# xiaohong-huang/RTK-Visual-Inertial-Navigation

Measured on AMD Instinct MI355X. Metric: gauss_newton_iterations_per_sec, higher is better.
Workload: dtype f64; 1 GPU; BASELINE cfg4: batch of 512 independent cfg3 windows (20 keyframes, 300 features, 3000 observations, 19 IMU factors, 10 satellites x 20 epochs carrier-phase+pseudorange, gauge prior) over the job, 8 dogleg iterations per solve; windows=512, windows_rank0=512

## Files before the change

### rtk_visual_inertial_navigation_amd/build.py

```python
import os
import subprocess

HERE = os.path.dirname(os.path.abspath(__file__))
CSRC = os.path.join(HERE, "csrc")
LIB = os.path.join(HERE, "libswf_hip.so")
SOURCES = ["swf_engine.hip", "swf_plan.cpp", "swf_problem.cpp", "swf_producers.hip", "swf_gnss_epochs.cpp", "swf_lambda.hip", "swf_features.hip", "swf_fixprior.hip", "swf_phasescreen.hip", "swf_gnssepoch.hip", "swf_ddselect.hip", "swf_pnp.hip", "swf_trackreject.hip"]
HEADERS = ["swf_dev.h", "swf_records.h", "swf_plan.h", "swf_kernels.h", "swf_clique_mm.h", "swf_lmschur.h", "swf_chol_rr4.h", "swf_kernels2.h", "swf_kernels3.h", "swf_rootdev.h", "swf_kernels4.h", "swf_lambda.h", "swf_features.h", "swf_fixprior.h", "swf_gnss_range.h", "swf_phasescreen.h", "swf_gnssepoch.h", "swf_ddselect.h", "swf_pnp.h", "swf_trackreject.h",
           os.path.join("..", "..", "include", "swf_types.h"),
           os.path.join("..", "..", "include", "swf_solver.h")]


def hipcc():
    for p in (os.environ.get("HIPCC"), "/opt/rocm/bin/hipcc", "hipcc"):
        if p and (os.path.isabs(p) and os.path.exists(p) or not os.path.isabs(p)):
            return p
    return "hipcc"


def needs_build():
    if not os.path.exists(LIB):
        return True
    t = os.path.getmtime(LIB)
    for f in SOURCES + HEADERS:
        p = os.path.join(CSRC, f)
        if os.path.exists(p) and os.path.getmtime(p) > t:
            return True
    return False


def build(force=False, verbose=False):
# ... 14 lines not shown
```

### rtk_visual_inertial_navigation_amd/csrc/swf_engine.hip

```cpp
#include <hip/hip_runtime.h>
#include <algorithm>
#include <chrono>
#include <cmath>
#include <cstdio>
#include <cstdlib>
#include <cstring>
#include <string>
#include <memory>
#include <thread>
#include <vector>
#include "../../include/swf_solver.h"
#include "swf_kernels2.h"
#include "swf_kernels3.h"
#include "swf_kernels4.h"
#include "swf_lambda.h"
#include "swf_ddselect.h"
#include "swf_features.h"
#include "swf_fixprior.h"
#include "swf_plan.h"

static thread_local std::string g_err;
static int fail(int code, const std::string& msg) { g_err = msg; return code; }
#define HIPCHK(x) do { hipError_t e_ = (x); if (e_ != hipSuccess) return fail(SWF_E_NODEVICE, std::string(#x) + ": " + hipGetErrorString(e_)); } while (0)

// ... 186 lines not shown
    std::vector<double> h_fxA, h_fxb, h_fxJ, h_fxr0, h_fxeig, h_fxx0; std::vector<int> h_fxrank, h_fxapplied;
    bool fc_built = false, fc_valid = false, fc_host = false; FeatArgs fc{}; char* fc_out = nullptr; size_t fc_bytes = 0; int fc_nfeat = 0;
    std::vector<int> fc_feat0; std::vector<char> h_fc;
    hipStream_t aux = nullptr; hipEvent_t ev_fork[3] = { nullptr, nullptr, nullptr };
    ~swf_batch() {
        if (aux) { (void)hipStreamSynchronize(aux); handle_cache().give(aux); }
        for (auto& e : ev_fork) handle_cache().give(e, false);
    }
    WinState* ws_primary = nullptr; WinState* ws_alt = nullptr; WinState* ws_alt2 = nullptr;
    bool no_decide_fuse = false;
    bool no_step_fuse = false;
    int n_pch_split = 0;
    bool no_spec = false;
    bool no_comp_fuse = false;
    bool lat_fuse = false;
    bool rr4_has15 = false, rr4_has16 = false;
    int rr_nmax = 256;
    bool L_full = false;
    int asm_programs = 0;
    int ls_qpb = 1, ls_var = 0, ls_kms = 8; bool ls_folded = false, s_direct = false;
    bool full_final = false;
    bool no_clq_pack = false;
    bool no_clq_mfma = false;
    int clp_rows = 1, clp_ld = 3;
    int ls_gqpb = 4;
    int timing = 0;
    swf_timing last{};
    std::vector<hipEvent_t> ev;
    std::vector<int> ev_kind;
    int ev_used = 0;
    int64_t jac_bytes = 0, proj_bytes = 0, chol_flops = 0, lm_schur_flops = 0, lm_schur_flops_sym = 0, lm_schur_mfma = 0;
    int last_mode = -1;
};

extern "C" int swf_batch_create(const swf_flat_window* const* windows, int32_t n, void* stream, swf_batch** out) {
    if (!windows || n <= 0 || !out) return fail(SWF_E_INVALID, "swf_batch_create: bad arguments");
    int ndev = 0;
    if (hipGetDeviceCount(&ndev) != hipSuccess || ndev <= 0)
        return fail(SWF_E_NODEVICE, "no HIP device: this library has no CPU fallback");
    int n_cu = 256;
    { int dev = 0; hipDeviceProp_t pr; if (hipGetDevice(&dev) == hipSuccess && hipGetDeviceProperties(&pr, dev) == hipSuccess && pr.multiProcessorCount > 0) n_cu = pr.multiProcessorCount; }
    Plan B;
    {
        std::string err;
        int prc = plan_build(windows, n, plan_shape_from_env(n_cu), B, err);
        if (prc != SWF_OK) return fail(prc, err);
    }
    std::unique_ptr<swf_batch> owner(new swf_batch());
    swf_batch* b = owner.get();
    b->device = current_device();
    b->stream = (hipStream_t)stream;
    b->n_cu = n_cu;
    b->no_comp_fuse = getenv("SWF_NO_COMP_FUSE") != nullptr;
    b->no_spec = getenv("SWF_NO_SPEC_EVAL") != nullptr;
    b->no_step_fuse = getenv("SWF_NO_STEP_FUSE") != nullptr;
    b->no_decide_fuse = getenv("SWF_NO_DECIDE_FUSE") != nullptr;
    b->full_final = getenv("SWF_FULL_FINAL_ELIM") != nullptr;
    b->no_clq_pack = getenv("SWF_NO_CLIQUE_PACK") != nullptr;
    b->no_clq_mfma = getenv("SWF_NO_CLIQUE_MFMA") != nullptr;
    b->max_tiles = B.max_tiles; b->max_prior_dim = B.max_prior_dim; b->max_red = B.max_red; b->min_red = B.min_red;
    b->rr_nmax = B.rr_nmax; b->rr4_has15 = B.rr4_has15; b->rr4_has16 = B.rr4_has16; b->n_pch_split = B.n_pch_split;
    b->lat_fuse = B.lat_fuse; b->asm_programs = B.asm_programs;
    b->ls_qpb = B.ls_qpb; b->ls_var = B.ls_var; b->ls_kms = B.ls_kms; b->ls_gqpb = B.ls_gqpb; b->ls_folded = B.ls_folded; b->s_direct = B.s_direct;
    for (int k = 0; k < 5; k++) b->clc_imu[k] = B.clc_imu[k];
    b->clp_rows = B.clp_rows; b->clp_ld = B.clp_ld;
    b->n_comp = B.n_comp; b->comp_nmax = B.comp_nmax; b->comp_nmin = B.comp_nmin; b->comp_ne = B.comp_ne;
    b->jac_bytes = B.jac_bytes; b->proj_bytes = B.proj_bytes; b->chol_flops = B.chol_flops;
    b->lm_schur_flops = B.lm_schur_flops; b->lm_schur_flops_sym = B.lm_schur_flops_sym; b->lm_schur_mfma = B.lm_schur_mfma;
    if (B.want_aux) {
        bool ok = (b->aux = handle_cache().stream()) != nullptr;
        for (int i = 0; i < 3 && ok; i++) ok = (b->ev_fork[i] = handle_cache().event(false)) != nullptr;
        if (!ok) { handle_cache().give(b->aux); b->aux = nullptr; }
    }
    DevBatch& D = b->D;
    DevPool& P = b->pool;
    int rc = 0;
    D.n_win = n; D.n_x = (int)B.n_x; D.n_loc_total = (int)B.n_loc; D.max_iter_trace = SWF_MAX_TRACE; D.rr_nmax = B.rr_nmax;
    D.n_lmb = B.n_lmb; D.n_pch = B.n_pch; D.n_proj = B.n_proj; D.n_lm = B.n_lm; D.n_fr = B.n_fr; D.n_fsb = B.n_fsb;
    D.n_gf = (int)B.gf.size(); D.n_imu = (int)B.imu_gf.size(); D.n_sc = (int)B.sc_gf.size(); D.n_prior = (int)B.prior_gf.size(); D.n_idp = (int)B.idp_gf.size();
    D.n_cl = (int)B.cl.size(); D.n_pair = (int)B.pair.size(); D.n_pd = B.n_pd; D.n_po = B.n_po; D.n_cle = B.n_cle;
    for (int k = 0; k < 5; k++) D.n_clc[k] = B.n_clc[k];
    D.as_max_ne = B.as_max_ne; D.as_max_nv = B.as_max_nv;
#define PUT(field) rc |= P.put(B.field, &D.field)
    PUT(win);
    PUT(lmb_rec); PUT(pch_q); PUT(pch_r0); PUT(prior_nch);
    PUT(blk_xoff); PUT(blk_loc); PUT(blk_gs);
    PUT(loc2x); PUT(x_var);
    PUT(p_win); PUT(p_xpose); PUT(p_xex); PUT(p_xlm);
// ... 184 lines not shown
    if (!b) return fail(SWF_E_INVALID, "null batch");
    b->fc_valid = false; b->dd_valid = false;
    int n = b->D.n_x;
    hipLaunchKernelGGL(k_copy, dim3((n + 255) / 256), dim3(256), 0, b->stream, b->D.x, (const double*)b->D.x0, n);
    HIPCHK(hipGetLastError());
    if (b->n_comp) {
        HIPCHK(hipMemcpyAsync(b->CA.pose, b->co_pose0, (size_t)b->comp_ne * 7 * sizeof(double), hipMemcpyDeviceToDevice, b->stream));
        HIPCHK(hipMemcpyAsync(b->CA.sb, b->co_sb0, (size_t)b->comp_ne * 9 * sizeof(double), hipMemcpyDeviceToDevice, b->stream));
        HIPCHK(hipMemsetAsync(b->CA.history, 0, (size_t)b->n_comp * sizeof(int), b->stream));
    }
    return SWF_OK;
}

static DevOpt to_devopt(const swf_options* o) {
    DevOpt d{};
    d.max_iter = o->max_num_iterations; d.step_mode = o->step_mode; d.strategy = o->trust_region_strategy; d.jacobi = o->jacobi_scaling ? 1 : 0;
    d.r0 = o->initial_trust_region_radius; d.max_r = o->max_trust_region_radius; d.min_r = o->min_trust_region_radius;
    d.min_rel_dec = o->min_relative_decrease; d.ftol = o->function_tolerance; d.gtol = o->gradient_tolerance;
    d.ptol = o->parameter_tolerance; d.min_mu = o->min_mu; d.max_mu = o->max_mu; d.mu_inc = o->mu_increase_factor;
    d.min_diag = o->min_diagonal; d.max_diag = o->max_diagonal;
    return d;
}

#define GRID(n, per) dim3((unsigned)(((n) + (per) - 1) / (per)))
namespace {
struct Launcher {
    swf_batch* b; DevOpt O; hipStream_t st;
    bool lm_folded = false;
    bool export_full = false;
    int lm_next = 0, lm_qpb = 1;
    int ls_tiles_per_launch() const { return b->ls_var == 0 ? 16 : b->ls_var == 1 ? 40 : 72; }
    WinState* ws_next(WinState* p) const { return p == b->ws_primary ? b->ws_alt : p == b->ws_alt ? b->ws_alt2 : b->ws_primary; }
    bool decide_fused = false;
    void lm_launch(int tile_base, hipStream_t on, int clique_rows = 0) {
        DevBatch& D = b->D;
        dim3 grid(D.n_win, GEMM_SPLIT / b->ls_qpb);
        const int qpb = b->ls_qpb, sd = b->s_direct ? 1 : 0, lp = tile_base / ls_tiles_per_launch(), kms = b->ls_kms;
        if (clique_rows > 0) {
            const int np = (int)grid.y;
            grid.y += clique_rows;
            if (decide_fused) {
                WinState* out = ws_next(D.ws);
                if (b->ls_var == 0) hipLaunchKernelGGL((k_decide_lm_clique<8, 2, 2, 80>), grid, dim3(LS_NT(8, 2)), 0, on, D, O, qpb, lp, kms, sd, np, out);
                else hipLaunchKernelGGL((k_decide_lm_clique<8, 5, 2, 144>), grid, dim3(LS_NT(8, 2)), 0, on, D, O, qpb, lp, kms, sd, np, out);
                D.ws = out;
                return;
// ... 128 lines not shown
                hipLaunchKernelGGL((k_lm_schur<8, 2, 2, 80, false, true>), grid, dim3(256), 0, st, D, O, b->ls_gqpb, 0, 0, 0);
            } else if (!write_S) {
                dim3 grid(D.n_win, GEMM_SPLIT / lm_qpb);
                hipLaunchKernelGGL((k_lm_schur<8, 2, 2, 80, false>), grid, dim3(256), 0, st, D, O, lm_qpb, 0, 0, 0);
            } else {
                const int crow = D.n_win > 0 ? (D.n_clc[2] + D.n_win - 1) / D.n_win : 0;
                clq_fused = clq_fuse_ok();
                lm_launch(0, st, clq_fused ? crow : 0);
                lm_next = ls_tiles_per_launch();
            }
        }
        {
            hipStream_t sa = b->aux ? b->aux : st;
            if (b->aux) (void)hipStreamWaitEvent(b->aux, b->ev_fork[1], 0);
            auto cstream = [&](int cls) { return (b->aux && !b->clc_imu[cls]) ? st : sa; };
            if (comp_fused) {
                for (; lm_next < b->max_tiles; lm_next += ls_tiles_per_launch()) { Bracket t(*this, SWF_K_LM_SCHUR, sa); lm_launch(lm_next, sa); }
            } else {
            const bool grad = !write_S && !b->full_final;
            if (D.n_clc[1]) {
                Bracket t(*this, SWF_K_CLIQUE_ELIM, cstream(1));
                if (grad) hipLaunchKernelGGL((k_clique_elim<32, 48, 9, 1, true>), dim3(D.n_clc[1]), dim3(64), 0, cstream(1), D, O);
                else if (b->no_clq_mfma) hipLaunchKernelGGL((k_clique_elim<32, 48, 9, 1>), dim3(D.n_clc[1]), dim3(64), 0, cstream(1), D, O);
                else hipLaunchKernelGGL((k_clique_mm<32, 48, 9>), dim3(D.n_clc[1]), dim3(64), 0, cstream(1), D, O);
            }
            if (D.n_clc[0]) {
                Bracket t(*this, SWF_K_CLIQUE_ELIM, cstream(0));
                constexpr int CLP_NW = 1;
                const size_t lds = CLP_NW * 2 * ((size_t)(b->clp_rows + 2) * b->clp_ld + b->clp_rows + 2) * sizeof(double);
                const dim3 cgrid(((D.n_clc[0] + 1) / 2 + CLP_NW - 1) / CLP_NW);
                if (b->no_clq_pack) {
                    if (grad) hipLaunchKernelGGL((k_clique_elim<48, 32, 1, 0, true>), dim3(D.n_clc[0]), dim3(64), 0, cstream(0), D, O);
                    else hipLaunchKernelGGL((k_clique_elim<48, 32, 1, 0>), dim3(D.n_clc[0]), dim3(64), 0, cstream(0), D, O);
                }
                else if (grad) hipLaunchKernelGGL((k_clique_pack<true, CLP_NW>), cgrid, dim3(64 * CLP_NW), lds, cstream(0), D, O, b->clp_rows, b->clp_ld);
                else hipLaunchKernelGGL((k_clique_pack<false, CLP_NW>), cgrid, dim3(64 * CLP_NW), lds, cstream(0), D, O, b->clp_rows, b->clp_ld);
            }
            if (D.n_clc[2] && !clq_fused) {
                Bracket t(*this, SWF_K_CLIQUE_ELIM, cstream(2));
                if (b->lat_fuse) {
                    if (grad) hipLaunchKernelGGL(k_clique_elim4<true>, dim3(D.n_clc[2]), dim3(256), 0, cstream(2), D, O);
                    else hipLaunchKernelGGL(k_clique_elim4<false>, dim3(D.n_clc[2]), dim3(256), 0, cstream(2), D, O);
                }
                else if (grad) hipLaunchKernelGGL((k_clique_elim<64, 64, 9, 2, true>), dim3(D.n_clc[2]), dim3(64), 0, cstream(2), D, O);
                else hipLaunchKernelGGL((k_clique_elim<64, 64, 9, 2>), dim3(D.n_clc[2]), dim3(64), 0, cstream(2), D, O);
            }
// ... 963 lines not shown
    }
    if (!ok) return fail(SWF_E_NODEVICE, "download failed");
    return SWF_OK;
}

extern "C" int swf_debug_plan_check(const swf_flat_window* const* windows, int32_t n, int32_t n_cu, int32_t ls_variant, int32_t ls_qpb, int32_t ls_grad_qpb,
                                    int32_t flags, int32_t corrupt_table, int32_t corrupt_index, int32_t* info) {
    if (!windows || n <= 0 || n_cu <= 0) return fail(SWF_E_INVALID, "swf_debug_plan_check: bad arguments");
    PlanShape sh;
    sh.n_cu = n_cu; sh.ls_variant = ls_variant; sh.ls_qpb = ls_qpb; sh.ls_grad_qpb = ls_grad_qpb; sh.no_lat_fuse = flags & 1; sh.no_chol_col = flags & 2;
    Plan B; std::string err;
    int rc = plan_build(windows, n, sh, B, err);
    if (rc != SWF_OK) return fail(rc, err);
    if (corrupt_table) {
        const size_t i = (size_t)corrupt_index;
        if (corrupt_table == 1 && i < B.as_src.size()) B.as_src[i] += 1 << 28;
        else if (corrupt_table == 2 && i < B.sch_rec.size()) B.sch_rec[i] ^= 1;
        else if (corrupt_table == 3 && i < B.s_tnz.size() && B.s_tnz[i]) B.s_tnz[i] &= B.s_tnz[i] - 1;
        else if (corrupt_table == 4 && i < B.prior_colloc.size()) B.prior_colloc[i] ^= 1;
        else if (corrupt_table == 5 && i < B.loc2x.size()) B.loc2x[i] ^= 1;
        else if (corrupt_table == 6 && i < B.co_voff.size()) B.co_voff[i] += 1 << 28;
        else if (corrupt_table == 7 && i < B.pair_o.size()) B.pair_o[i].q_base += 8;
        else if (corrupt_table == 8 && i < B.imu_rec.size()) B.imu_rec[i].xo[3] ^= 1;
        else return fail(SWF_E_INVALID, "swf_debug_plan_check: nothing to corrupt there");
    }
    if (info) {
        const int v[12] = { B.ls_var, B.ls_qpb, B.ls_gqpb, B.ls_folded, B.lat_fuse, B.want_aux, B.want_Linv, B.want_Wk, B.asm_programs, B.n_pch_split, B.max_red, B.n_pch };
        for (int k = 0; k < 12; k++) info[k] = v[k];
    }
    rc = plan_validate(B, err);
    return rc == SWF_OK ? SWF_OK : fail(rc, err);
}

extern "C" int swf_debug_mfma_f64(const double* A, const double* Bm, const double* C, double* D) {
    if (!A || !Bm || !C || !D) return fail(SWF_E_INVALID, "swf_debug_mfma_f64: bad arguments");
    double* dv = nullptr;
    if (hipMalloc(&dv, (64 + 64 + 256 + 256) * sizeof(double)) != hipSuccess) return fail(SWF_E_NODEVICE, "swf_debug_mfma_f64: allocation failed");
    bool ok = hipMemcpy(dv, A, 64 * sizeof(double), hipMemcpyHostToDevice) == hipSuccess
        && hipMemcpy(dv + 64, Bm, 64 * sizeof(double), hipMemcpyHostToDevice) == hipSuccess
        && hipMemcpy(dv + 128, C, 256 * sizeof(double), hipMemcpyHostToDevice) == hipSuccess;
    if (ok) {
        hipLaunchKernelGGL(k_debug_mfma_f64, dim3(1), dim3(64), 0, 0, dv, dv + 64, dv + 128, dv + 384);
        ok = hipGetLastError() == hipSuccess && hipMemcpy(D, dv + 384, 256 * sizeof(double), hipMemcpyDeviceToHost) == hipSuccess;
    }
    (void)hipFree(dv);
    return ok ? SWF_OK : fail(SWF_E_NODEVICE, "swf_debug_mfma_f64: the device run failed");
}

#ifdef SWF_PROFILE_CHOL
extern "C" int swf_debug_chol_stamps(unsigned long long* out) {
    if (hipDeviceSynchronize() != hipSuccess) return SWF_E_NODEVICE;
    if (hipMemcpyFromSymbol(out, HIP_SYMBOL(g_chol_stamps), 64 * sizeof(unsigned long long)) != hipSuccess) return SWF_E_NODEVICE;
    return SWF_OK;
}
#endif

#ifdef SWF_PROFILE_CHOLW
extern "C" int swf_debug_chol_wstep(int step) {
    if (hipDeviceSynchronize() != hipSuccess) return SWF_E_NODEVICE;
    unsigned long long z[16 * 8] = { 0 };
    if (hipMemcpyToSymbol(HIP_SYMBOL(g_chol_wst), z, sizeof(z)) != hipSuccess) return SWF_E_NODEVICE;
    if (hipMemcpyToSymbol(HIP_SYMBOL(g_chol_wstep), &step, sizeof(int)) != hipSuccess) return SWF_E_NODEVICE;
    return SWF_OK;
}
extern "C" int swf_debug_chol_wstamps(unsigned long long* out) {
    if (hipDeviceSynchronize() != hipSuccess) return SWF_E_NODEVICE;
    if (hipMemcpyFromSymbol(out, HIP_SYMBOL(g_chol_wst), 16 * 8 * sizeof(unsigned long long)) != hipSuccess) return SWF_E_NODEVICE;
    return SWF_OK;
}
// ... 175 lines not shown
```

### rtk_visual_inertial_navigation_amd/csrc/swf_kernels.h

```cpp
#pragma once
#include "swf_dev.h"

struct DevOpt {
    int max_iter, step_mode, strategy, jacobi;
    double r0, max_r, min_r, min_rel_dec, ftol, gtol, ptol, min_mu, max_mu, mu_inc, min_diag, max_diag;
};



__device__ __forceinline__ double damp_diag(const DevOpt& O, double d, double* jsc_slot, bool first) {
    if (!O.jacobi) return clampd(d, O.min_diag, O.max_diag);
    double q;
    if (first) { double r = 1.0 + sqrt(d > 0.0 ? d : 0.0); q = r * r; *jsc_slot = q; }
    else q = *jsc_slot;
    return clampd(d / q, O.min_diag, O.max_diag) * q;
}

__device__ __forceinline__ double pinned_d(double v) { asm volatile("" : "+v"(v)); return v; }
template <bool JAC> __device__ __forceinline__ bool eval_gate(const DevBatch& B, const WinState& s) { return B.spec == 2 ? true : (JAC && !B.spec) ? s.need_lin != 0 : s.eval_cand != 0; }
template <bool JAC> __device__ __forceinline__ const double* eval_src(const DevBatch& B) { return (JAC && !B.spec) ? B.x : B.xc; }

#include "swf_gnss_range.h"

template <bool JAC, bool STORE>
// ... 1056 lines not shown
            }
#pragma unroll
            for (int u = 0; u < 2; u++) {
                if (!on[u]) continue;
                int i = i0[u], j = j0[u];
                bool i1ok = i + 1 < df, j1ok = j + 1 < df;
                Cm[i * df + j] = m[u][0]; Cm[j * df + i] = m[u][0];
                if (i1ok) { Cm[(i + 1) * df + j] = m[u][2]; Cm[j * df + i + 1] = m[u][2]; }
                if (!diag[u] && j1ok) { Cm[i * df + j + 1] = m[u][1]; Cm[(j + 1) * df + i] = m[u][1]; }
                if (i1ok && j1ok) { Cm[(i + 1) * df + j + 1] = m[u][3]; Cm[(j + 1) * df + i + 1] = m[u][3]; }
            }
        }
    }
    QST(5);
}
template <int MAXR, int MAXD, int MAXE, int CLS, bool GRAD = false>
__global__ void __launch_bounds__(64) k_clique_elim(DevBatch B, DevOpt O) { d_clique_elim<MAXR, MAXD, MAXE, CLS, 24, 1, 4, GRAD>(B, O, (int)blockIdx.x); }
template <bool GRAD = false>
__global__ void __launch_bounds__(256) k_clique_elim4(DevBatch B, DevOpt O) { d_clique_elim<64, 64, 9, 2, 8, 4, 4, GRAD>(B, O, (int)blockIdx.x); }
template <bool GRAD = false>
__global__ void __launch_bounds__(256) k_clique_tall(DevBatch B, DevOpt O) { d_clique_elim<CLQ_TALLR, 64, 9, 4, 8, 4, 4, GRAD>(B, O, (int)blockIdx.x); }

#include "swf_clique_mm.h"

__device__ __forceinline__ double readhalf_d(double v, bool upper) { double a = readlane_d(v, 0), b = readlane_d(v, 32); return upper ? b : a; }
template <bool GRAD, int NW>
__global__ void __launch_bounds__(64 * NW) k_clique_pack(DevBatch B, DevOpt O, const int R, const int LD) {
    constexpr int PF = 12;
    extern __shared__ double clp_lds[];
    const int lane = threadIdx.x & 63, hl = lane & 31, pair = (int)blockIdx.x * NW + (NW > 1 ? __builtin_amdgcn_readfirstlane((int)threadIdx.x >> 6) : 0);
    const bool up = lane >= 32;
    double* Jc = clp_lds + (2 * (pair - (int)blockIdx.x * NW) + (up ? 1 : 0)) * ((R + 2) * LD + R + 2);
    double* rv = Jc + R * LD; double* Me = rv + R; double* T = Me + LD; double* Ei = T + LD; double* Eg = Ei + 1;
    const int n = B.n_clc[0];
    int cidx = 2 * pair + (up ? 1 : 0);
    bool act = cidx < n;
    const Clique& C = B.clc_rec[0][act ? cidx : 0];
    WinState& s = B.ws[C.win];
    act = act && s.need_lin;
    if (__builtin_amdgcn_ballot_w64(act) == 0) return;
    const int de = act ? C.d_e : 0, df = act ? C.d_f : 0, d = de + df, nrow = act ? C.n_rows : 0, tot = nrow * d;
    const int nrow_m = max(__builtin_amdgcn_readlane(nrow, 0), __builtin_amdgcn_readlane(nrow, 32));
    const int tot_m = max(__builtin_amdgcn_readlane(tot, 0), __builtin_amdgcn_readlane(tot, 32));
    {
        const double* gJ = B.g_J + C.j_off;
        float rd = 1.0f / (float)(nrow > 0 ? nrow : 1);
// ... 412 lines not shown
```

### rtk_visual_inertial_navigation_amd/csrc/swf_plan.cpp

```cpp
#include <algorithm>
#include <array>
#include <cstdlib>
#include <cstring>
#include <map>
#include <string>
#include <vector>
#include "swf_plan.h"

namespace {
int refuse(std::string& err, int code, const std::string& msg) { err = msg; return code; }
int ls_ncw(int var) { return var <= 1 ? 8 : 12; }
int ls_tpw(int var) { return var == 0 ? 2 : var == 1 ? 5 : 6; }

int plan_window(Plan& B, const swf_flat_window* w, int wi, HostWin& hw, std::string& err) {
    WinRec R{};
    const int nP = w->n_pose, nS = w->n_sb, nL = w->n_lm, nC = w->n_sc;
    const int nb = nP + nS + nL + nC;
    if (nb <= 0) return refuse(err, SWF_E_INVALID, "empty window");
    hw = HostWin{ w->pose, w->sb, w->lm, w->sc, nP, nS, nL, nC, 0 };
    R.x_base = (int)B.n_x; R.blk_base = (int)B.blk_xoff.size(); R.n_blk = nb;
    R.loc_base = (int)B.n_loc;
    std::vector<int> gs(nb), ls(nb), xo(nb), loc(nb, -1), grp(nb, -1);
    int xoff = 0;
    for (int b = 0; b < nb; b++) {
// ... 717 lines not shown
    std::stable_sort(po.begin(), po.end(), [&](int a, int c) {
        return (B.pair[a].la * B.pair[a].lb + 15) / 16 > (B.pair[c].la * B.pair[c].lb + 15) / 16; });
    for (size_t i = 0; i < B.cl.size(); i++) {
        const Clique& c = B.cl[i];
        if (c.d_e > 0) cle.push_back((int)i);
        if (c.is_static) continue;
        int d = c.d_e + c.d_f;
        int cls = (c.d_e <= 1 && d <= 32 && c.n_rows <= 48) ? 0 : (c.n_rows <= 32 && d <= 48) ? 1 : (c.n_rows <= CLQ_MAXR && d <= CLQ_MAXD) ? 2 : (c.n_rows <= CLQ_TALLR && d <= 64) ? 4 : 3;
        if (B.lat_fuse && cls < 2) cls = 2;
        clc[cls].push_back((int)i);
        for (int q = c.fac0; q < c.fac1; q++) if (B.gf[B.cl_fac[q]].type == GF_IMU) B.clc_imu[cls] = true;
    }
    B.n_pd = (int)pd.size(); B.n_po = (int)po.size(); B.n_cle = (int)cle.size();
    std::vector<Pair>&vd = B.pair_d, &vo = B.pair_o;
    for (int i : pd) vd.push_back(B.pair[i]);
    for (int i : po) vo.push_back(B.pair[i]);
    for (int i : cle) B.cle_rec.push_back(B.cl[i]);
    for (int k = 0; k < 5; k++) {
        for (int i : clc[k]) B.clc_rec[k].push_back(B.cl[i]);
        B.n_clc[k] = (int)clc[k].size();
    }
    B.clp_rows = 1; B.clp_ld = 3;
    for (const Clique& c : B.clc_rec[0]) { B.clp_rows = std::max(B.clp_rows, c.n_rows); B.clp_ld = std::max(B.clp_ld, (c.d_e + c.d_f + 2) | 1); }
}

int plan_asm_programs(Plan& B, const std::vector<int>& pd, const std::vector<int>& po, std::string& err) {
    const int n_part = B.s_direct ? 0 : B.ls_folded ? 1 : GEMM_SPLIT, n_qpart = B.ls_folded ? 1 : GEMM_SPLIT;
    const int n = B.n_win;
    struct Prog { std::vector<int> dst, src0, aux, src, vloc, vred, vsrc0, vi, vsrc; std::vector<unsigned> cnt, vcnt; };
    std::vector<AsmWin>& asw = B.asw;
    asw.assign((size_t)n, AsmWin{});
    std::vector<int>&t_dst = B.as_dst, &t_src0 = B.as_src0, &t_aux = B.as_aux, &t_src = B.as_src, &tv_loc = B.av_loc, &tv_red = B.av_red, &tv_src0 = B.av_src0, &tv_i = B.av_i, &tv_src = B.av_src;
    std::vector<unsigned>&t_cnt = B.as_cnt, &tv_cnt = B.av_cnt;
    std::map<std::vector<int>, std::array<int, 4>> seen;
    std::vector<std::vector<int>> wpairs((size_t)n);
    for (int i : pd) wpairs[(size_t)B.pair[i].win].push_back(i);
    for (int i : po) wpairs[(size_t)B.pair[i].win].push_back(i);
    bool overflow = false;
    std::vector<unsigned>& tnz = B.s_tnz;
    tnz.assign((size_t)n * 4, 0u);
    for (const Pair& Pq : B.pair) {
        if (B.win[(size_t)Pq.win].n_red > 256) continue;
        for (int I = Pq.ra / 16; I <= (Pq.ra + Pq.la - 1) / 16; I++)
            for (int J = Pq.rb / 16; J <= (Pq.rb + Pq.lb - 1) / 16 && J < I; J++) { const int t = I * (I - 1) / 2 + J; tnz[(size_t)Pq.win * 4 + (t >> 5)] |= 1u << (t & 31); }
    }
    for (int w = 0; w < n; w++) {
// ... 293 lines not shown
        }
        if (!C.is_static) cl_seen[{ C.fac0, C.mem0, C.e_off }] = 0;
    }
    for (int k = 0; k < 5; k++) {
        NEED((int)B.clc_rec[k].size() == B.n_clc[k], "clc_rec", k);
        for (const Clique& C : B.clc_rec[k]) {
            const long long d = C.d_e + C.d_f; const int R = C.n_rows;
            auto it = cl_seen.find({ C.fac0, C.mem0, C.e_off });
            NEED(it != cl_seen.end() && it->second++ == 0, "clc_rec", k);
            NEED(k == 0 ? (C.d_e <= 1 && d <= 32 && R <= 48) : k == 1 ? (R <= 32 && d <= 48) : k == 2 ? (R <= CLQ_MAXR && d <= CLQ_MAXD) : k == 4 ? (R <= CLQ_TALLR && d <= 64)
                        : (d <= CB_MAXD && C.d_e <= 9 && (long long)C.d_e * d <= CB_MAXED), "clc_rec", k);
        }
    }
    for (auto& kv : cl_seen) NEED(kv.second == 1, "clc_rec: a clique in no class, fac0", kv.first[0]);
    NEED(B.clp_rows >= 1 && B.clp_rows <= 48 && B.clp_ld >= 3 && B.clp_ld <= 35 && (B.clp_ld & 1) == 1, "clp_rows", B.clp_rows);
    {
        int mr = 1, ml = 3;
        for (const Clique& C : B.clc_rec[0]) {
            NEED(C.n_rows <= B.clp_rows && C.d_e + C.d_f + 2 <= B.clp_ld, "clp_ld", &C - B.clc_rec[0].data());
            mr = std::max(mr, C.n_rows); ml = std::max(ml, (C.d_e + C.d_f + 2) | 1);
        }
        NEED(mr == B.clp_rows && ml == B.clp_ld, "clp_rows: not the largest class-0 clique", mr);
    }
    const int TW = B.ls_var <= 1 ? 2 : 1, NCW = ls_ncw(B.ls_var), TPW = ls_tpw(B.ls_var);
    NEED((long long)B.sch_rec.size() >= ((long long)B.sch_c0.back() + 4 * LS_NB) * 32 && (long long)B.sch_km.size() >= ((long long)B.sch_c0.back() / TW + 2) * B.ls_kms, "sch_rec", B.sch_rec.size());
    std::vector<std::vector<const Pair*>> wpair((size_t)n);
    auto pair_ok = [&](const Pair& P) {
        if (!in(P.win, 0, n)) return false;
        const WinRec& W = B.win[P.win];
        return P.ra >= 0 && P.la >= 1 && P.ra + P.la <= W.n_red && P.rb >= 0 && P.lb >= 1 && P.rb + P.lb <= W.n_red && P.rb <= P.ra && in(P.fa, -1, W.nF) && in(P.fb, -1, W.nF)
            && P.c0 >= 0 && P.c0 <= P.c1 && P.c1 <= (long long)B.pc_coff.size() && (P.is_diag ? (P.ra == P.rb && P.la == P.lb) : P.ra != P.rb) && P.loc_a == W.loc_base + W.n_e + P.ra
            && P.fsb0 == W.fsb0 && P.fsb1 == W.fsb1 && P.n == W.n_red && P.m == 6 * W.nF && P.S_base == W.S_base && P.P_base == W.P_base && P.q_base == 6LL * W.fr_base * GEMM_SPLIT;
    };
    NEED((int)B.pair_d.size() == B.n_pd && (int)B.pair_o.size() == B.n_po, "pair_d", B.pair_d.size());
    for (const Pair& P : B.pair) NEED(pair_ok(P), "pair", &P - B.pair.data());
    for (const Pair& P : B.pair_d) { NEED(pair_ok(P) && P.is_diag, "pair_d", &P - B.pair_d.data()); wpair[P.win].push_back(&P); }
    for (const Pair& P : B.pair_o) { NEED(pair_ok(P) && !P.is_diag, "pair_o", &P - B.pair_o.data()); wpair[P.win].push_back(&P); }
    std::map<std::array<int, 4>, std::vector<int>> programs;
    for (int w = 0; w < n; w++) {
        const WinRec& W = B.win[w];
        NEED(W.n_e + W.n_red == W.n_loc && W.loc_base >= 0 && W.loc_base + W.n_loc <= B.n_loc && W.x_base >= 0 && W.x_base + W.x_n <= B.n_x, "win", w);
        NEED(W.S_base >= 0 && W.S_base + (long long)(W.n_red + 1) * W.n_red <= B.S_tot && W.Lt_base + (long long)(W.n_red + 1) * (W.n_red + 1) <= B.Lt_tot && W.P_base + 36LL * W.nF * W.nF <= B.P_tot, "win", w);
        NEED(W.fr_base >= 0 && W.fr_base + W.nF <= B.n_fr && W.nF <= LS_MAXF && W.lm0 <= W.lm1 && W.lm1 <= B.n_lm, "win", w);
        for (int f = 0; f < W.nF; f++) NEED(B.fr_red[W.fr_base + f] >= 0 && B.fr_red[W.fr_base + f] + 6 <= W.n_red, "fr_red", W.fr_base + f);
        {
            int l = W.lm0;
// ... 89 lines not shown
```

### rtk_visual_inertial_navigation_amd/csrc/swf_plan.h

```cpp
#pragma once
#include <string>
#include <vector>
#include "../../include/swf_solver.h"
#include "swf_records.h"

struct FeatWinSrc {
    int x_base = 0, n_pose = 0, n_sb = 0, n_lm = 0, n_sc = 0;
    std::vector<int> proj_idx; std::vector<double> proj_uv;
    std::vector<int> idp_kind, idp_idx; std::vector<double> idp_pts;
    double pbg[3] = { 0, 0, 0 }; double sqrt_info = 0;
};

struct HostWin {
    double *pose, *sb, *lm, *sc;
    int n_pose, n_sb, n_lm, n_sc;
    int tail_dim;
    double *comp_pose = nullptr, *comp_sb = nullptr;
    int comp_e0 = 0, comp_ne = 0;
    std::vector<int> p_orig;
    int n_proj_all = 0;
    std::vector<int> tail_x;
    FeatWinSrc feat;
    struct LinPrior { int gf, dim, gsum; std::vector<int> col_x; };
    std::vector<LinPrior> lin_prior;
// ... 42 lines not shown
    int max_tiles = 0, max_prior_dim = 0;
    std::vector<int> lmb_rec, pch_q, pch_r0, prior_nch;
    std::vector<int> sch_c0, sch_rec, sch_km;
    std::vector<int> fsb_rec;
    std::vector<JtRec> sc_jt, imu_jt;
    std::vector<ImuRec> imu_rec;
    std::vector<double> prior_Jt;
    std::vector<int> prior_colloc, prior_colcc, s_pcol, s_pxo, cv_loc;
    std::vector<Pair> pair_d, pair_o;
    std::vector<Clique> clc_rec[5], cle_rec;
    std::vector<AsmWin> asw;
    std::vector<unsigned> s_tnz;
    std::vector<int> as_dst, as_src0, as_aux, as_src, av_loc, av_red, av_src0, av_i, av_src;
    std::vector<unsigned> as_cnt, av_cnt;
    std::vector<int> co_eo, co_no, co_roff, co_x0off, co_voff, co_iq_f, co_iq_k;
    std::vector<long long> co_pno, co_nno, co_go, co_g2o, co_Joff, co_Coff;
    int n_win = 0, n_proj = 0, n_lm = 0, n_lmb = 0, n_pch = 0, n_fsb = 0, n_pd = 0, n_po = 0, n_cle = 0, n_clc[5] = { 0, 0, 0, 0, 0 };
    int as_max_ne = 0, as_max_nv = 0;
    int n_cu = 256, rr_nmax = 256, max_red = 0, min_red = 1 << 30;
    int ls_qpb = 1, ls_var = 0, ls_kms = 8, ls_gqpb = 4; bool ls_folded = false, s_direct = false;
    bool lat_fuse = false, want_aux = false, want_Linv = false, want_Wk = false;
    bool clc_imu[5] = { false, false, false, false, false };
    int clp_rows = 1, clp_ld = 3;
    int n_pch_split = 0; bool rr4_has15 = false, rr4_has16 = false;
    int n_comp = 0, comp_nmax = 0, comp_nmin = 1 << 30; long long comp_ne = 0;
    int asm_programs = 0;
    int64_t jac_bytes = 0, proj_bytes = 0, chol_flops = 0, lm_schur_flops = 0, lm_schur_flops_sym = 0, lm_schur_mfma = 0;
};

int plan_build(const swf_flat_window* const* windows, int n, const PlanShape& shape, Plan& plan, std::string& err);

int plan_validate(const Plan& plan, std::string& err);
```

Before: 733,300 iterations/s.

## Add direct class-1 clique elimination kernel using augmented-column MFMA Gram

Adds k_clique_md, a class-1 clique elimination kernel that appends the residual as an extra column. One set of f64 MFMA passes then yields both the Gram matrix and the gradient. It inverts the eliminated block in registers with a lane-broadcast Gauss-Jordan and applies the Schur update with MFMA into the same accumulators. The plan picks it when every class-1 clique has at most 47 columns, and an env var turns it off. The aim is fewer passes and less shared-memory traffic per clique, at the cost of extra register pressure and a second code path to keep correct.

```diff
diff --git a/rtk_visual_inertial_navigation_amd/build.py b/rtk_visual_inertial_navigation_amd/build.py
--- a/rtk_visual_inertial_navigation_amd/build.py
+++ b/rtk_visual_inertial_navigation_amd/build.py
@@ -5,7 +5,7 @@
 CSRC = os.path.join(HERE, "csrc")
 LIB = os.path.join(HERE, "libswf_hip.so")
 SOURCES = ["swf_engine.hip", "swf_plan.cpp", "swf_problem.cpp", "swf_producers.hip", "swf_gnss_epochs.cpp", "swf_lambda.hip", "swf_features.hip", "swf_fixprior.hip", "swf_phasescreen.hip", "swf_gnssepoch.hip", "swf_ddselect.hip", "swf_pnp.hip", "swf_trackreject.hip"]
-HEADERS = ["swf_dev.h", "swf_records.h", "swf_plan.h", "swf_kernels.h", "swf_clique_mm.h", "swf_lmschur.h", "swf_chol_rr4.h", "swf_kernels2.h", "swf_kernels3.h", "swf_rootdev.h", "swf_kernels4.h", "swf_lambda.h", "swf_features.h", "swf_fixprior.h", "swf_gnss_range.h", "swf_phasescreen.h", "swf_gnssepoch.h", "swf_ddselect.h", "swf_pnp.h", "swf_trackreject.h",
+HEADERS = ["swf_dev.h", "swf_records.h", "swf_plan.h", "swf_kernels.h", "swf_clique_mm.h", "swf_clique_md.h", "swf_lmschur.h", "swf_chol_rr4.h", "swf_kernels2.h", "swf_kernels3.h", "swf_rootdev.h", "swf_kernels4.h", "swf_lambda.h", "swf_features.h", "swf_fixprior.h", "swf_gnss_range.h", "swf_phasescreen.h", "swf_gnssepoch.h", "swf_ddselect.h", "swf_pnp.h", "swf_trackreject.h",
            os.path.join("..", "..", "include", "swf_types.h"),
            os.path.join("..", "..", "include", "swf_solver.h")]
 
diff --git a/rtk_visual_inertial_navigation_amd/csrc/swf_clique_md.h b/rtk_visual_inertial_navigation_amd/csrc/swf_clique_md.h
--- /dev/null
+++ b/rtk_visual_inertial_navigation_amd/csrc/swf_clique_md.h
@@ -0,0 +1,197 @@
+#pragma once
+
+template <int MAXR, int MAXD, int MAXE>
+__global__ void __launch_bounds__(64) k_clique_md(DevBatch B, DevOpt O) {
+    static_assert(MAXR % 4 == 0 && MAXD == 48 && MAXE <= 16, "k_clique_md: whole k-steps, three 16-column tiles, the eliminated block inside tile column 0");
+    static_assert(CMM_SLOT_ROW[0] == 0 && CMM_SLOT_ROW[1] == 1 && CMM_SLOT_ROW[2] == 2 && CMM_SLOT_ROW[3] == 3, "k_clique_md: slot kk of a k-step holds row k0 + kk");
+    constexpr int CLS = 1, KS = MAXR / 4, KE = (MAXE + 3) / 4;
+    __shared__ double lds[(2 * MAXD + MAXE + 1) * MAXE];
+    static_assert(MAXE * MAXE + MAXE >= MAXD, "k_clique_md: g is staged in the Ei | Eg region");
+    double (*Me)[MAXD] = reinterpret_cast<double (*)[MAXD]>(lds);
+    double (*T)[MAXD] = reinterpret_cast<double (*)[MAXD]>(lds + MAXE * MAXD);
+    double (*Ei)[MAXE] = reinterpret_cast<double (*)[MAXE]>(lds + 2 * MAXE * MAXD);
+    double* Eg = lds + 2 * MAXE * MAXD + MAXE * MAXE;
+    double* gs = lds + 2 * MAXE * MAXD;
+    const int cidx_ = (int)blockIdx.x;
+#ifdef SWF_PROFILE_CLQ
+    unsigned long long tq_ = __builtin_amdgcn_s_memtime();
+    if (cidx_ == SWF_PROFILE_CLQ_IDX && threadIdx.x == 0) for (int i = 0; i < 16; i++) g_clq_stamps[i] = 0;
+#endif
+    if (cidx_ >= B.n_clc[CLS]) return;
+    const Clique& C = B.clc_rec[CLS][cidx_];
+    WinState& s = B.ws[C.win];
+    const int lane = threadIdx.x, li = lane & 15, lk = lane >> 4;
+    const int de = C.d_e, df = C.d_f, d = de + df, nrow = C.n_rows, nr4 = (nrow + 3) & ~3;
+    const int nt = (d + 16) >> 4;
+    const double* gJ = B.g_J + C.j_off;
+    const double* gr = B.g_r + C.r_off;
+    const int need = s.need_lin;
+    const double s_mu = s.mu; const bool s_it0 = s.iter == 0;
+    double x[KS][3];
+#pragma unroll
+    for (int t = 0; t < 3; t++) {
+        const int col = 16 * t + li;
+        const double* p = col < d ? gJ + col * nrow : gr;
+#pragma unroll
+        for (int ks = 0; ks < KS; ks++) { const int row = 4 * ks + lk; x[ks][t] = (col <= d && row < nrow) ? p[row] : 0.0; }
+    }
+#pragma unroll
+    for (int ks = 0; ks < KS; ks++)
+#pragma unroll
+        for (int t = 0; t < 3; t++) x[ks][t] = pinned_d(x[ks][t]);
+    if (!need) return;
+    QST(0);
+    QST(1);
+    double4_t acc[6];
+#pragma unroll
+    for (int t = 0; t < 6; t++) acc[t] = double4_t{ 0, 0, 0, 0 };
+#pragma unroll
+    for (int ks = 0; ks < KS; ks++) {
+        if (4 * ks < nr4) {
+#pragma unroll
+            for (int ti = 0; ti < 3; ti++)
+#pragma unroll
+                for (int tj = 0; tj <= ti; tj++)
+                    if (ti < nt) acc[ti * (ti + 1) / 2 + tj] = __builtin_amdgcn_mfma_f64_16x16x4f64(x[ks][ti], x[ks][tj], acc[ti * (ti + 1) / 2 + tj], 0, 0, 0);
+        }
+    }
+    {
+        const int td = d >> 4, rd = d & 15;
+#pragma unroll
+        for (int tc = 0; tc < 3; tc++) {
+            if (tc <= td) {
+                double v = 0;
+#pragma unroll
+                for (int ti = tc; ti < 3; ti++)
+#pragma unroll
+                    for (int r = 0; r < 4; r++)
+                        if (ti == td && r == (rd >> 2)) v = acc[ti * (ti + 1) / 2 + tc][r];
+                if (lk == (rd & 3)) gs[16 * tc + li] = v;
+            }
+        }
+    }
+#pragma unroll
+    for (int ti = 0; ti < 3; ti++) {
+        if (ti < nt) {
+#pragma unroll
+            for (int r = 0; r < 4; r++) {
+                const int row = lk + 4 * r;
+                if (row == li) T[0][16 * ti + li] = acc[ti * (ti + 1) / 2 + ti][r];
+                if (li < MAXE) Me[li][16 * ti + row] = (li < de && 16 * ti + row != d) ? acc[ti * (ti + 1) / 2][r] : 0.0;
+            }
+        }
+    }
+    __syncthreads();
+    const double gc = gs[lane < d ? lane : 0];
+    if (lane < d) {
+        const double mcc = T[0][lane];
+        if (lane < de) { B.g[C.e_loc + lane] = gc; B.diag[C.e_loc + lane] = mcc; B.vc[C.e_loc + lane] = gc / clampd(mcc, O.min_diag, O.max_diag); }
+        else { B.cv_graw[C.v_off + lane - de] = gc; B.cv_dgraw[C.v_off + lane - de] = mcc; }
+    }
+    __syncthreads();
+    QST(2);
+    if (de > 0) {
+        {
+            double row[2 * MAXE];
+#pragma unroll
+            for (int j = 0; j < MAXE; j++) {
+                double v = (lane < de && j < de) ? Me[lane][j] : 0.0;
+                if (j == lane) v += s_mu * (lane < de ? damp_diag(O, v, B.jsc + C.e_loc + lane, s_it0) : clampd(v, O.min_diag, O.max_diag));
+                row[j] = v; row[MAXE + j] = (j == lane) ? 1.0 : 0.0;
+            }
+            bool bad = false;
+#pragma unroll
+            for (int k = 0; k < MAXE; k++) {
+                if (k < de) {
+                    double piv = readlane_d(row[k], k);
+                    if (!(piv > 0.0)) bad = true;
+                    double ip = __builtin_amdgcn_rcp(piv);
+                    ip = ip * (2.0 - piv * ip); ip = ip * (2.0 - piv * ip);
+                    double aik = row[k];
+#pragma unroll
+                    for (int j = 0; j < 2 * MAXE; j++) {
+                        double akj = readlane_d(row[j], k) * ip;
+                        row[j] = (lane == k) ? akj : row[j] - aik * akj;
+                    }
+                }
+            }
+            if (bad) { if (lane == 0) s.lin_fail = 1; return; }
+            if (lane < MAXE) {
+#pragma unroll
+                for (int j = 0; j < MAXE; j++) Ei[lane][j] = (lane < de && j < de) ? row[MAXE + j] : 0.0;
+            }
+        }
+        __syncthreads();
+        QST(3);
+        {
+            double gE = 0;
+            int j = lane < df ? lane : 0;
+            double mcol[MAXE], gb[MAXE];
+#pragma unroll
+            for (int b2 = 0; b2 < MAXE; b2++) { mcol[b2] = Me[b2][de + j]; gb[b2] = readlane_d(gc, b2); }
+#pragma unroll 1
+            for (int a2 = 0; a2 < MAXE; a2++) {
+                double sv = 0, sg = 0;
+#pragma unroll
+                for (int b2 = 0; b2 < MAXE; b2++) { double ev = Ei[a2][b2]; sv += ev * mcol[b2]; sg += ev * gb[b2]; }
+                if (lane < df) T[a2][lane] = sv;
+                if (lane == a2) gE = sg;
+            }
+            if (lane < de) Eg[lane] = gE;
+        }
+        __syncthreads();
+        QST(4);
+        double* E = B.cE + C.e_off;
+        {
+            for (int e = lane; e < de * de; e += 64) E[e] = Ei[e / de][e % de];
+            if (lane < df) {
+#pragma unroll
+                for (int a2 = 0; a2 < MAXE; a2++) if (a2 < de) E[de * de + a2 * df + lane] = Me[a2][de + lane];
+            }
+            if (lane < de) E[de * de + de * df + lane] = gc;
+            if (lane < df) {
+                double v = 0;
+#pragma unroll
+                for (int a2 = 0; a2 < MAXE; a2++) v -= Me[a2][de + lane] * (a2 < de ? Eg[a2] : 0.0);
+                B.cv_cs[C.v_off + lane] = v;
+            }
+        }
+#pragma unroll
+        for (int ks = 0; ks < KE; ks++) {
+            const int a2 = 4 * ks + lk, a2c = a2 < MAXE ? a2 : 0;
+            double fa[3], tb[3];
+#pragma unroll
+            for (int t = 0; t < 3; t++) {
+                const int cc = 16 * t + li - de;
+                const bool on = t < nt && a2 < MAXE;
+                fa[t] = on ? -Me[a2c][16 * t + li] : 0.0;
+                tb[t] = on && cc >= 0 && cc < df ? T[a2c][cc] : 0.0;
+            }
+#pragma unroll
+            for (int ti = 0; ti < 3; ti++)
+#pragma unroll
+                for (int tj = 0; tj <= ti; tj++)
+                    if (ti < nt) acc[ti * (ti + 1) / 2 + tj] = __builtin_amdgcn_mfma_f64_16x16x4f64(fa[ti], tb[tj], acc[ti * (ti + 1) / 2 + tj], 0, 0, 0);
+        }
+    } else {
+        if (lane < df) B.cv_cs[C.v_off + lane] = 0.0;
+    }
+    double* Cm = B.C + C.C_off;
+#pragma unroll
+    for (int ti = 0; ti < 3; ti++)
+#pragma unroll
+        for (int tj = 0; tj <= ti; tj++) {
+            if (ti < nt) {
+#pragma unroll
+                for (int r = 0; r < 4; r++) {
+                    const int R = 16 * ti + lk + 4 * r, Cc = 16 * tj + li;
+                    if (R >= Cc && Cc >= de && R < d) {
+                        const int i = R - de, j = Cc - de;
+                        const double v = acc[ti * (ti + 1) / 2 + tj][r];
+                        Cm[i * df + j] = v; Cm[j * df + i] = v;
+                    }
+                }
+            }
+        }
+    QST(5);
+}
diff --git a/rtk_visual_inertial_navigation_amd/csrc/swf_engine.hip b/rtk_visual_inertial_navigation_amd/csrc/swf_engine.hip
--- a/rtk_visual_inertial_navigation_amd/csrc/swf_engine.hip
+++ b/rtk_visual_inertial_navigation_amd/csrc/swf_engine.hip
@@ -232,6 +232,8 @@
     bool full_final = false;
     bool no_clq_pack = false;
     bool no_clq_mfma = false;
+    bool no_clq_direct = false;
+    bool clq_direct = true;
     int clp_rows = 1, clp_ld = 3;
     int ls_gqpb = 4;
     int timing = 0;
@@ -268,12 +270,13 @@
     b->full_final = getenv("SWF_FULL_FINAL_ELIM") != nullptr;
     b->no_clq_pack = getenv("SWF_NO_CLIQUE_PACK") != nullptr;
     b->no_clq_mfma = getenv("SWF_NO_CLIQUE_MFMA") != nullptr;
+    b->no_clq_direct = getenv("SWF_NO_CLIQUE_DIRECT") != nullptr;
     b->max_tiles = B.max_tiles; b->max_prior_dim = B.max_prior_dim; b->max_red = B.max_red; b->min_red = B.min_red;
     b->rr_nmax = B.rr_nmax; b->rr4_has15 = B.rr4_has15; b->rr4_has16 = B.rr4_has16; b->n_pch_split = B.n_pch_split;
     b->lat_fuse = B.lat_fuse; b->asm_programs = B.asm_programs;
     b->ls_qpb = B.ls_qpb; b->ls_var = B.ls_var; b->ls_kms = B.ls_kms; b->ls_gqpb = B.ls_gqpb; b->ls_folded = B.ls_folded; b->s_direct = B.s_direct;
     for (int k = 0; k < 5; k++) b->clc_imu[k] = B.clc_imu[k];
-    b->clp_rows = B.clp_rows; b->clp_ld = B.clp_ld;
+    b->clp_rows = B.clp_rows; b->clp_ld = B.clp_ld; b->clq_direct = B.clq_direct;
     b->n_comp = B.n_comp; b->comp_nmax = B.comp_nmax; b->comp_nmin = B.comp_nmin; b->comp_ne = B.comp_ne;
     b->jac_bytes = B.jac_bytes; b->proj_bytes = B.proj_bytes; b->chol_flops = B.chol_flops;
     b->lm_schur_flops = B.lm_schur_flops; b->lm_schur_flops_sym = B.lm_schur_flops_sym; b->lm_schur_mfma = B.lm_schur_mfma;
@@ -504,6 +507,8 @@
     return d;
 }
 
+static bool clique_direct(bool no_clq_direct, bool all_below_48) { return !no_clq_direct && all_below_48; }
+
 #define GRID(n, per) dim3((unsigned)(((n) + (per) - 1) / (per)))
 namespace {
 struct Launcher {
@@ -678,6 +683,7 @@
                 Bracket t(*this, SWF_K_CLIQUE_ELIM, cstream(1));
                 if (grad) hipLaunchKernelGGL((k_clique_elim<32, 48, 9, 1, true>), dim3(D.n_clc[1]), dim3(64), 0, cstream(1), D, O);
                 else if (b->no_clq_mfma) hipLaunchKernelGGL((k_clique_elim<32, 48, 9, 1>), dim3(D.n_clc[1]), dim3(64), 0, cstream(1), D, O);
+                else if (clique_direct(b->no_clq_direct, b->clq_direct)) hipLaunchKernelGGL((k_clique_md<32, 48, 9>), dim3(D.n_clc[1]), dim3(64), 0, cstream(1), D, O);
                 else hipLaunchKernelGGL((k_clique_mm<32, 48, 9>), dim3(D.n_clc[1]), dim3(64), 0, cstream(1), D, O);
             }
             if (D.n_clc[0]) {
@@ -1687,6 +1693,7 @@
         else if (corrupt_table == 6 && i < B.co_voff.size()) B.co_voff[i] += 1 << 28;
         else if (corrupt_table == 7 && i < B.pair_o.size()) B.pair_o[i].q_base += 8;
         else if (corrupt_table == 8 && i < B.imu_rec.size()) B.imu_rec[i].xo[3] ^= 1;
+        else if (corrupt_table == 9 && i == 0) B.clq_direct = !B.clq_direct;
         else return fail(SWF_E_INVALID, "swf_debug_plan_check: nothing to corrupt there");
     }
     if (info) {
@@ -1710,6 +1717,56 @@
     }
     (void)hipFree(dv);
     return ok ? SWF_OK : fail(SWF_E_NODEVICE, "swf_debug_mfma_f64: the device run failed");
+}
+
+extern "C" int swf_debug_plan_clique_direct(const swf_flat_window* const* windows, int32_t n, int32_t n_cu, int32_t flags) {
+    if (!windows || n <= 0 || n_cu <= 0) return fail(SWF_E_INVALID, "swf_debug_plan_clique_direct: bad arguments");
+    PlanShape sh;
+    sh.n_cu = n_cu; sh.no_lat_fuse = flags & 1; sh.no_chol_col = flags & 2;
+    Plan B; std::string err;
+    int rc = plan_build(windows, n, sh, B, err);
+    if (rc != SWF_OK) return fail(rc, err);
+    return B.clq_direct ? 1 : 0;
+}
+
+extern "C" int swf_debug_clique_out_doubles(int32_t d_e, int32_t d_f) { return 3 * d_e + 3 * d_f + (d_e * d_e + d_e * d_f + d_e) + d_f * d_f + d_e; }
+extern "C" int swf_debug_clique(int32_t form, int32_t n_rows, int32_t d_e, int32_t d_f, const double* J, const double* r, double mu, int32_t iter,
+                                const double* jsc, int32_t jacobi, int32_t need_lin, double fill, double* out, int32_t* lin_fail, int32_t* ran) {
+    const int d = d_e + d_f;
+    if (!J || !r || !out || !lin_fail || !ran || (d_e > 0 && !jsc) || form < 0 || form > 2 || n_rows < 1 || n_rows > 32 || d_e < 0 || d_e > 9 || d_f < 1 || d > 48)
+        return fail(SWF_E_INVALID, "swf_debug_clique: bad arguments");
+    const bool direct = form == 2 ? clique_direct(getenv("SWF_NO_CLIQUE_DIRECT") != nullptr, d <= 47) : form == 1;
+    if (direct && d > 47) return fail(SWF_E_INVALID, "swf_debug_clique: k_clique_md has no spare column for a clique of 48 columns");
+    const size_t nJ = (size_t)n_rows * d, nout = (size_t)swf_debug_clique_out_doubles(d_e, d_f);
+    std::vector<double> h(nJ + n_rows + nout, fill);
+    std::copy(J, J + nJ, h.begin()); std::copy(r, r + n_rows, h.begin() + nJ);
+    if (d_e > 0) std::copy(jsc, jsc + d_e, h.end() - d_e);
+    WinState ws{}; ws.mu = mu; ws.iter = iter; ws.need_lin = need_lin;
+    Clique cq{}; cq.d_e = d_e; cq.d_f = d_f; cq.n_rows = n_rows;
+    double* dv = nullptr; WinState* dws = nullptr; Clique* dcq = nullptr;
+    bool ok = hipMalloc(&dv, h.size() * sizeof(double)) == hipSuccess && hipMalloc(&dws, sizeof(WinState)) == hipSuccess && hipMalloc(&dcq, sizeof(Clique)) == hipSuccess
+        && hipMemcpy(dv, h.data(), h.size() * sizeof(double), hipMemcpyHostToDevice) == hipSuccess
+        && hipMemcpy(dws, &ws, sizeof(WinState), hipMemcpyHostToDevice) == hipSuccess && hipMemcpy(dcq, &cq, sizeof(Clique), hipMemcpyHostToDevice) == hipSuccess;
+    if (ok) {
+        swf_options o; swf_default_options(&o); o.jacobi_scaling = jacobi ? 1 : 0;
+        const DevOpt O = to_devopt(&o);
+        DevBatch D{};
+        D.n_win = 1; D.ws = dws; D.n_clc[1] = 1; D.clc_rec[1] = dcq; D.g_J = dv; D.g_r = dv + nJ;
+        double* p = dv + nJ + n_rows;
+        D.g = p; D.diag = p + d_e; D.vc = p + 2 * d_e; p += 3 * d_e;
+        D.cv_graw = p; D.cv_dgraw = p + d_f; D.cv_cs = p + 2 * d_f; p += 3 * d_f;
+        D.cE = p; p += d_e * d_e + d_e * d_f + d_e;
+        D.C = p; p += d_f * d_f;
+        D.jsc = p;
+        if (direct) hipLaunchKernelGGL((k_clique_md<32, 48, 9>), dim3(1), dim3(64), 0, 0, D, O);
+        else hipLaunchKernelGGL((k_clique_mm<32, 48, 9>), dim3(1), dim3(64), 0, 0, D, O);
+        ok = hipGetLastError() == hipSuccess && hipMemcpy(out, dv + nJ + n_rows, nout * sizeof(double), hipMemcpyDeviceToHost) == hipSuccess
+            && hipMemcpy(&ws, dws, sizeof(WinState), hipMemcpyDeviceToHost) == hipSuccess;
+    }
+    (void)hipFree(dv); (void)hipFree(dws); (void)hipFree(dcq);
+    if (!ok) return fail(SWF_E_NODEVICE, "swf_debug_clique: the device run failed");
+    *lin_fail = ws.lin_fail; *ran = direct ? 1 : 0;
+    return SWF_OK;
 }
 
 #ifdef SWF_PROFILE_CHOL
diff --git a/rtk_visual_inertial_navigation_amd/csrc/swf_kernels.h b/rtk_visual_inertial_navigation_amd/csrc/swf_kernels.h
--- a/rtk_visual_inertial_navigation_amd/csrc/swf_kernels.h
+++ b/rtk_visual_inertial_navigation_amd/csrc/swf_kernels.h
@@ -1102,6 +1102,7 @@
 __global__ void __launch_bounds__(256) k_clique_tall(DevBatch B, DevOpt O) { d_clique_elim<CLQ_TALLR, 64, 9, 4, 8, 4, 4, GRAD>(B, O, (int)blockIdx.x); }
 
 #include "swf_clique_mm.h"
+#include "swf_clique_md.h"
 
 __device__ __forceinline__ double readhalf_d(double v, bool upper) { double a = readlane_d(v, 0), b = readlane_d(v, 32); return upper ? b : a; }
 template <bool GRAD, int NW>
diff --git a/rtk_visual_inertial_navigation_amd/csrc/swf_plan.cpp b/rtk_visual_inertial_navigation_amd/csrc/swf_plan.cpp
--- a/rtk_visual_inertial_navigation_amd/csrc/swf_plan.cpp
+++ b/rtk_visual_inertial_navigation_amd/csrc/swf_plan.cpp
@@ -763,6 +763,8 @@
     }
     B.clp_rows = 1; B.clp_ld = 3;
     for (const Clique& c : B.clc_rec[0]) { B.clp_rows = std::max(B.clp_rows, c.n_rows); B.clp_ld = std::max(B.clp_ld, (c.d_e + c.d_f + 2) | 1); }
+    B.clq_direct = true;
+    for (const Clique& c : B.clc_rec[1]) if (c.d_e + c.d_f > 47) B.clq_direct = false;
 }
 
 int plan_asm_programs(Plan& B, const std::vector<int>& pd, const std::vector<int>& po, std::string& err) {
@@ -1102,6 +1104,11 @@
         }
         NEED(mr == B.clp_rows && ml == B.clp_ld, "clp_rows: not the largest class-0 clique", mr);
     }
+    {
+        int md = 0;
+        for (const Clique& C : B.clc_rec[1]) md = std::max(md, C.d_e + C.d_f);
+        NEED(B.clq_direct == (md <= 47), "clq_direct: not what the widest class-1 clique says", md);
+    }
     const int TW = B.ls_var <= 1 ? 2 : 1, NCW = ls_ncw(B.ls_var), TPW = ls_tpw(B.ls_var);
     NEED((long long)B.sch_rec.size() >= ((long long)B.sch_c0.back() + 4 * LS_NB) * 32 && (long long)B.sch_km.size() >= ((long long)B.sch_c0.back() / TW + 2) * B.ls_kms, "sch_rec", B.sch_rec.size());
     std::vector<std::vector<const Pair*>> wpair((size_t)n);
diff --git a/rtk_visual_inertial_navigation_amd/csrc/swf_plan.h b/rtk_visual_inertial_navigation_amd/csrc/swf_plan.h
--- a/rtk_visual_inertial_navigation_amd/csrc/swf_plan.h
+++ b/rtk_visual_inertial_navigation_amd/csrc/swf_plan.h
@@ -88,6 +88,7 @@
     bool lat_fuse = false, want_aux = false, want_Linv = false, want_Wk = false;
     bool clc_imu[5] = { false, false, false, false, false };
     int clp_rows = 1, clp_ld = 3;
+    bool clq_direct = true;
     int n_pch_split = 0; bool rr4_has15 = false, rr4_has16 = false;
     int n_comp = 0, comp_nmax = 0, comp_nmin = 1 << 30; long long comp_ne = 0;
     int asm_programs = 0;
```

Result: no change. 738,400 iterations/s (median of 3 runs) (+0.7%).
